# lanl-ansi/Katana.jl

Hardware: AMD Instinct MI355X
Metric: ECP iterations/sec + wall-clock to f_tol=1e-6, 1e5-var synthetic convex NLP (higher is better)
Workload: dtype f64; 1 GPU; cfg3: n=100000 variables, m_lin=50000 linear rows (8 nnz), m_nl=10000 explog rows (k=32 nnz), seed 0, planted non-degenerate vertex optimum, f_tol=1e-6; parallelism=1 GPU

## Files before the change

katana.jl_amd/csrc/engine.hpp:

```cpp
#pragma once
#include <hip/hip_runtime.h>

#include <algorithm>
#include <chrono>
#include <cstdlib>
#include <cmath>
#include <limits>
#include <map>
#include <string>
#include <vector>

#include <rccl/rccl.h>

#include "common.hpp"
#include "types.hpp"
#include "prims.hpp"

namespace ktn {

static const double kInf = std::numeric_limits<double>::infinity();

static inline int pick_group(double avg_len) {
    int g = 4;
    while (g < 64 && 2 * g <= avg_len) g <<= 1;
// ... 20 lines not shown
    int quad_group = 0;
    int esh_quad_group = 0;
    int ecp_quad_group = 0;
    int tiled_wg = 2;
    int ecp_power = 20;
    int grp_rows = 0, grp_cols = 0;
    int tiled = -1;
    double smax_reuse = 0.0;
    int power_passes = 0;
    int omega_robust = 1;
    int packed_trips = 0;
    int first_chunk = 31;
    int stag_chunk = 0;
    int near_chunk = -1;
    int stag_checks = 2;
    double flat_factor = 0.4;
    int omega_art = 1;
    double omega_art_k = 256.0;
    double omega_art_clamp = 0.0, omega_clamp = 0.0, omega_clamp_down = 0.0;
    double ipc_timeout_s = 20.0;
    bool raw_duals = false;
    int mid_refactor = 0;
    int kkt_group = 0;
    static bool flag(const char* k) { return std::getenv(k) != nullptr; }
    static int geti(const char* k, int d) { const char* v = std::getenv(k); return v ? std::atoi(v) : d; }
    static double getd(const char* k, double d) { const char* v = std::getenv(k); return v ? std::atof(v) : d; }
    void from_env() {
        no_pinned_check = flag("KTN_NO_PINNED_CHECK"); debug_load = flag("KTN_DEBUG_LOAD"); no_csc_merge = flag("KTN_NO_CSC_MERGE");
        tiled_general_build = flag("KTN_TILED_GENERAL_BUILD"); debug_blocks = flag("KTN_DEBUG_BLOCKS"); no_tiled_check = flag("KTN_NO_TILED_CHECK");
        no_setup_reuse = flag("KTN_NO_SETUP_REUSE"); debug_lp = flag("KTN_DEBUG_LP"); no_packed = flag("KTN_NO_PACKED");
        force_collective = flag("KTN_FORCE_COLLECTIVE");
        sweep_rows = geti("KTN_SWEEP_ROWS", sweep_rows); blk_cfg = geti("KTN_BLK_CFG", blk_cfg); sweep_blocked = geti("KTN_SWEEP_BLOCKED", sweep_blocked);
        sweep_batched = geti("KTN_SWEEP_BATCHED", sweep_batched); tape_classed = geti("KTN_TAPE_CLASSED", tape_classed);
        quad_group = geti("KTN_QUAD_GROUP", quad_group); esh_quad_group = geti("KTN_ESH_QUAD_GROUP", esh_quad_group);
        ecp_quad_group = geti("KTN_ECP_QUAD_GROUP", ecp_quad_group);
        tiled_wg = geti("KTN_TILED_WG", tiled_wg); ecp_power = geti("KTN_ECP_POWER", ecp_power);
        grp_rows = geti("KTN_GRP_ROWS", grp_rows); grp_cols = geti("KTN_GRP_COLS", grp_cols); tiled = geti("KTN_TILED", tiled);
        smax_reuse = getd("KTN_SMAX_REUSE", smax_reuse); power_passes = geti("KTN_POWER_PASSES", power_passes);
        omega_robust = geti("KTN_OMEGA_ROBUST", omega_robust); packed_trips = geti("KTN_PACKED_TRIPS", packed_trips);
        first_chunk = geti("KTN_FIRST_CHUNK", first_chunk); stag_chunk = geti("KTN_STAG_CHUNK", stag_chunk); near_chunk = geti("KTN_NEAR_CHUNK", near_chunk);
        stag_checks = geti("KTN_STAG_CHECKS", stag_checks); flat_factor = getd("KTN_FLAT_FACTOR", flat_factor);
        omega_art = geti("KTN_OMEGA_ART", omega_art); omega_art_k = getd("KTN_OMEGA_ART_K", omega_art_k);
        omega_art_clamp = getd("KTN_OMEGA_ART_CLAMP", omega_art_clamp); omega_clamp = getd("KTN_OMEGA_CLAMP", omega_clamp);
        omega_clamp_down = getd("KTN_OMEGA_CLAMP_DOWN", omega_clamp_down); ipc_timeout_s = getd("KTN_IPC_TIMEOUT_S", ipc_timeout_s);
        mid_refactor = geti("KTN_MID_REFACTOR", mid_refactor); raw_duals = flag("KTN_RAW_DUALS");
        kkt_group = geti("KTN_KKT_GROUP", kkt_group);
    }
};

struct Engine {
    ktn_params prm;
    DevParams dev;
    std::string err;
    hipStream_t stream = nullptr;
    int device = 0;

    bool loaded = false;
    int64_t n0 = 0, m0 = 0;
    int64_t n_lp = 0;
    int64_t m_ext = 0;
    int64_t nnz_ext = 0;
    int sense = KTN_MIN;
    bool obj_linear = true;
    bool has_inf_bound = false;
    bool has_big_bound = false;
    std::vector<int64_t> h_rowptr;
    std::vector<int32_t> h_col;
    std::vector<uint8_t> h_rowkind;
    std::vector<double> h_lb, h_ub;
// ... 410 lines not shown
    bool kkt_solved = false, kkt_arena = false, kkt_cached = false, kkt_mirror = false, kkt_seg_ok = false;
    uint64_t kkt_solves = 0, kkt_key_version = 0, kkt_key_solves = 0;
    DBuf<int32_t> d_kkt_rowmap;
    int64_t kkt_n_lin = 0;
    DBuf<int64_t> d_kkt_cptr, d_kkt_seg;
    DBuf<int32_t> d_kkt_crow, d_kkt_nonfin;
    DBuf<uint32_t> d_kkt_cperm;
    DBuf<double> d_kkt_x, d_kkt_g, d_kkt_jac, d_kkt_bconst, d_kkt_maxc, d_kkt_d, d_kkt_z, d_kkt_t, d_kkt_out, d_kkt_blk;
    std::vector<double> h_kkt_d, h_kkt_z, h_kkt_blk;
    double kkt_bound = 0.0, kkt_gap = 0.0;
    bool kkt_foreign() const { return row_sharded() || dist.cb != nullptr || dist.comm != nullptr || dist.ipc.data != nullptr || exchanging(); }
    void kkt_build_mirror();
    void kkt_compute();
    void kkt_blocks();

    void rebuild_csc();
    void purge_cuts();
    void reserve_lp(int64_t rows, int64_t nnz);
    void find_long_rows();
    bool recession_ray_dense(bool* unbounded);
    void launch_y(const SpMat& A, double sigma, double w, double rho, hipEvent_t e0, hipEvent_t e1);
    void launch_x(const SpMat& AT, double tau, double w, double rho, bool update, hipEvent_t e0, hipEvent_t e1);
    void pdhg_iteration(const SpMat& A, const SpMat& AT, double tau, double sigma, double w, double rho);
    bool launch_check(const SpMat& A, const SpMat& AT, double tau, double sigma, double w_next = -1.0, double rho = 1.0);
    DBuf<double> xnext, ynext;
    int chk_nrow = 0, chk_ncol = 0;
    void compute_scaling(bool identity);
    LpResult lp_solve(double tol_p, double tol_g, int mode, bool identity_scaling = false);
    LpResult lp_solve_core(double tol_p, double tol_g, int mode, bool identity_scaling);
    bool lp_solve_dense(LpResult* R);
    bool big_bounds_hold();
    bool lp_solve_mid(LpResult* R);
    void pdhg_raw(const double* x0, const double* y0, double eta, double omega_, int64_t iters, double* x_out,
                  double* y_out);
    void lp_resize_iterates();
    void lp_pick_groups();
    void lp_choose_tiled(bool same_matrix);
    void lp_set_anchors(bool want_packed);
    void lp_read_check(double* q);
    void lp_restart();
    void lp_advance(bool spec, int64_t k, double rho);
    struct LpScriptIO {
        const double *x, *y, *x0, *y0;
        double eta, omega;
        int64_t k;
        int32_t flags;
        const int32_t* ops;
        int64_t nops;
// ... 17 lines not shown
```

katana.jl_amd/csrc/kernels.hpp:

```cpp
#pragma once
#include <hip/hip_runtime.h>

#include <cstdint>
#include <type_traits>

#include "../../include/katana_hip.h"
#include "types.hpp"

namespace ktn {

constexpr int kKindShift = 29;
constexpr int kColMask = (1 << kKindShift) - 1;

template <int G>
__device__ __forceinline__ double group_sum(double v) {
#pragma unroll
    for (int off = G / 2; off > 0; off >>= 1) v += __shfl_xor(v, off, 64);
    return v;
}
constexpr int kLaneU = 4;
template <int U>
struct LaneBatch {
    uint32_t ix[U];
    double v[U], g[U], h[U];
// ... 29 lines not shown
#pragma unroll
    for (int u = 0; u < U; ++u)
        if (b.on[u]) acc += b.v[u] * b.g[u];
}
template <int U>
__device__ __forceinline__ void lane_add2(const LaneBatch<U>& b, double& acc, double& acc2) {
#pragma unroll
    for (int u = 0; u < U; ++u)
        if (b.on[u]) { acc += b.v[u] * b.g[u]; acc2 += b.v[u] * b.h[u]; }
}
template <int G, int U = kLaneU, class E>
__device__ __forceinline__ void lane_dot(double& acc, E beg, E len, int lane, const int32_t* __restrict__ idx, const double* __restrict__ val,
                                         const double* __restrict__ vec, int from = 0) {
    const E end = beg + len;
    for (E left = len - from - lane; left > 0; left -= U * G) {
        LaneBatch<U> b;
        lane_load<G, U>(b, end - left, end, idx, val);
        lane_gather<U>(b, vec);
        lane_add<U>(b, acc);
    }
}
template <int G, int U = kLaneU, class E>
__device__ __forceinline__ void lane_dot2(double& acc, double& acc2, E beg, E len, int lane, const int32_t* __restrict__ idx,
                                          const double* __restrict__ val, const double* __restrict__ vec, const double* __restrict__ vec2) {
    const E end = beg + len;
    for (E left = len - lane; left > 0; left -= U * G) {
        LaneBatch<U> b;
        lane_load<G, U>(b, end - left, end, idx, val);
        lane_gather2<U>(b, vec, vec2);
        lane_add2<U>(b, acc, acc2);
    }
}

template <int G>
__device__ __forceinline__ double group_max(double v) {
#pragma unroll
    for (int off = G / 2; off > 0; off >>= 1) v = fmax(v, __shfl_xor(v, off, 64));
    return v;
}
template <int G>
__device__ __forceinline__ int group_or(int v) {
#pragma unroll
    for (int off = G / 2; off > 0; off >>= 1) v |= __shfl_xor(v, off, 64);
    return v;
}
__device__ __forceinline__ double nanmax(double a, double b) {
    return (a != a || b != b) ? __builtin_nan("") : (a > b ? a : b);
}
template <int G>
// ... 1035 lines not shown
struct __attribute__((aligned(32))) ColRec { double c, l, u, x0; };
struct __attribute__((aligned(32))) RowRec { double lo, hi, y0; int32_t beg, len; };

static __global__ __launch_bounds__(kBlock) void k_pack_both(int64_t n, const int64_t* __restrict__ cptr, const double* __restrict__ c,
                                                      const double* __restrict__ l, const double* __restrict__ u, const double* __restrict__ x,
                                                      double* __restrict__ x0, ColRec* __restrict__ crec, int2* __restrict__ bl, int64_t m,
                                                      const int64_t* __restrict__ rptr, const double* __restrict__ lo, const double* __restrict__ hi,
                                                      const double* __restrict__ y, double* __restrict__ y0, RowRec* __restrict__ rrec) {
    const int64_t i = (int64_t)blockIdx.x * kBlock + threadIdx.x;
    if (i < n) {
        const double xv = x[i];
        x0[i] = xv;
        ColRec r; r.c = c[i]; r.l = l[i]; r.u = u[i]; r.x0 = xv;
        crec[i] = r;
        bl[i] = make_int2((int)cptr[i], (int)(cptr[i + 1] - cptr[i]));
    }
    if (i < m) {
        const double yv = y[i];
        y0[i] = yv;
        RowRec r; r.lo = lo[i]; r.hi = hi[i]; r.y0 = yv; r.beg = (int32_t)rptr[i]; r.len = (int32_t)(rptr[i + 1] - rptr[i]);
        rrec[i] = r;
    }
}
template <int G, int T>
__global__ __launch_bounds__(kBlock) void k_pdhg_x_packed(int64_t n, const int2* __restrict__ bl, const int32_t* __restrict__ idx,
                                                          const double* __restrict__ val, const double* __restrict__ y,
                                                          double* __restrict__ x, double* __restrict__ xbar,
                                                          const ColRec* __restrict__ rec, double tau, double w, double rho) {
    const int64_t groups = (int64_t)gridDim.x * (kBlock / G);
    const int64_t g0 = ((int64_t)blockIdx.x * kBlock + threadIdx.x) / G;
    const int lane = threadIdx.x & (G - 1);
    int2 b[T];
    ColRec r[T];
    double xv[T], acc[T];
    LaneBatch<kLaneU> lb[T];
#pragma unroll
    for (int t = 0; t < T; ++t) {
        const int64_t j = g0 + t * groups;
        b[t] = (j < n) ? bl[j] : make_int2(0, 0);
        acc[t] = 0.0;
    }
#pragma unroll
    for (int t = 0; t < T; ++t) lane_load<G, kLaneU>(lb[t], b[t].x + lane, b[t].x + b[t].y, idx, val);
#pragma unroll
    for (int t = 0; t < T; ++t) {
        const int64_t j = g0 + t * groups;
        const bool on = j < n;
        if (on) r[t] = rec[j];
        xv[t] = on ? x[j] : 0.0;
    }
#pragma unroll
    for (int t = 0; t < T; ++t) lane_gather<kLaneU>(lb[t], y);
#pragma unroll
    for (int t = 0; t < T; ++t) lane_add<kLaneU>(lb[t], acc[t]);
#pragma unroll
    for (int t = 0; t < T; ++t) lane_dot<G>(acc[t], b[t].x, b[t].y, lane, idx, val, y, kLaneU * G);
#pragma unroll
    for (int t = 0; t < T; ++t) {
        const int64_t j = g0 + t * groups;
        const double a = group_sum<G>(acc[t]);
        if (lane == 0 && j < n) {
            const double xtv = prox_x(xv[t], tau, r[t].c, a, r[t].l, r[t].u);
            xbar[j] = 2.0 * xtv - xv[t];
            x[j] = halpern(w, rho, xtv, xv[t], r[t].x0);
        }
    }
}
template <int G, int T>
__global__ __launch_bounds__(kBlock) void k_pdhg_y_packed(int64_t m, const int32_t* __restrict__ idx, const double* __restrict__ val,
                                                          const double* __restrict__ xbar, double* __restrict__ y,
                                                          const RowRec* __restrict__ rec, double sigma, double w, double rho,
                                                          int long_thresh, const int32_t* __restrict__ long_rows, int n_long) {
    const int nreg = (int)gridDim.x - n_long;
    if ((int)blockIdx.x >= nreg) {
        __shared__ double sh[kBlock / 64];
        const int i = long_rows[(int)blockIdx.x - nreg];
        const RowRec rr = rec[i];
        const int end = rr.beg + rr.len;
        double acc = 0.0;
        int e = rr.beg + (int)threadIdx.x;
        for (; e + 15 * kBlock < end; e += 16 * kBlock) {
            double v[16], xg[16];
#pragma unroll
            for (int k = 0; k < 16; ++k) v[k] = val[e + k * kBlock];
#pragma unroll
            for (int k = 0; k < 16; ++k) xg[k] = xbar[idx[e + k * kBlock]];
#pragma unroll
            for (int k = 0; k < 16; ++k) acc += v[k] * xg[k];
        }
// ... 272 lines not shown
    double xtv = 0.0, xv = 0.0, x0v = 0.0, cj = 0.0, lj = 0.0, uj = 0.0, dcj = 1.0;
    if (on) { xtv = xt[j]; xv = x[j]; x0v = x0[j]; cj = c[j]; lj = l[j]; uj = u[j]; dcj = dc[j]; }
    double aty = 0.0;
    lane_dot<G>(aty, beg, end - beg, lane, AT.idx, AT.val, yt);
    aty = group_sum<G>(aty);
    if (on && lane == 0) {
        chk_col_accumulate(a, xtv, xv, x0v, aty, cj, lj, uj, dcj);
    }
    chk_block_store<kBlock, kChkColMask, G>(a, partials);
}

template <bool UPDATE>
__global__ __launch_bounds__(kBlock) void k_x_prox(int64_t n, const double* __restrict__ aty, double* __restrict__ x,
                                                   const double* __restrict__ x0, double* __restrict__ xt, double* __restrict__ xbar,
                                                   const double* __restrict__ c, const double* __restrict__ l,
                                                   const double* __restrict__ u, double tau, double w, double rho) {
    const int64_t j = (int64_t)blockIdx.x * kBlock + threadIdx.x;
    if (j >= n) return;
    const double xv = x[j];
    const double xtv = prox_x(xv, tau, c[j], aty[j], l[j], u[j]);
    if (UPDATE) { xbar[j] = 2.0 * xtv - xv; x[j] = halpern(w, rho, xtv, xv, x0[j]); }
    else xt[j] = xtv;
}
static __global__ __launch_bounds__(kBlock) void k_chk_cols_vec(int64_t n, const double* __restrict__ atyv, const double* __restrict__ x,
                                                         const double* __restrict__ xt, const double* __restrict__ x0,
                                                         const double* __restrict__ c, const double* __restrict__ l,
                                                         const double* __restrict__ u, const double* __restrict__ dc,
                                                         double* __restrict__ partials) {
    const int64_t j = (int64_t)blockIdx.x * kBlock + threadIdx.x;
    ChkAcc a; a.init();
    if (j < n) {
        const double xtv = xt[j], xv = x[j], x0v = x0[j], cj = c[j], lj = l[j], uj = u[j], dcj = dc[j], aty = atyv[j];
        chk_col_accumulate(a, xtv, xv, x0v, aty, cj, lj, uj, dcj);
    }
    chk_block_store<kBlock, kChkColMask>(a, partials);
}

__device__ __forceinline__ double ipc_load(const double* p) {
    return __longlong_as_double((long long)__hip_atomic_load((unsigned long long*)p, __ATOMIC_RELAXED, __HIP_MEMORY_SCOPE_SYSTEM));
}
static __global__ __launch_bounds__(64) void k_ipc_barrier(IpcPeers P, int rank, int world, unsigned long long epoch, long long timeout_ticks,
                                                    int* __restrict__ err) {
    constexpr unsigned long long kPoison = ~0ULL;
    const int t = threadIdx.x;
    if (t >= world) return;
    volatile int* verr = err;
// ... 937 lines not shown
```

katana.jl_amd/csrc/lp.hip:

```cpp
#include "engine.hpp"
#include "launch.hpp"
#include "kernels.hpp"
#include "pdhg_check.hpp"
#include "dense_lp.hpp"
#include "mid_lp.hpp"
#include "batch_lp.hpp"

namespace ktn {

double Engine::dev_dot(int64_t n, const double* a, const double* b) {
    launch(k_dot_partial, kRedBlocks, kBlock, 0, stream, n, a, b, partials.p);
    launch(k_sum_final, 1, kRedBlocks, 0, stream, partials.p, kRedBlocks, chkout.p + 2 * kChkQ);
    double v = 0.0;
    KTN_HIP(hipMemcpyAsync(&v, chkout.p + 2 * kChkQ, sizeof(double), hipMemcpyDeviceToHost, stream));
    sync();
    return v;
}

double Engine::dev_finite_sq(int64_t n, const double* a) {
    launch(k_finite_sq_partial, kRedBlocks, kBlock, 0, stream, n, a, partials.p);
    launch(k_sum_final, 1, kRedBlocks, 0, stream, partials.p, kRedBlocks, chkout.p + 2 * kChkQ);
    double v = 0.0;
    KTN_HIP(hipMemcpyAsync(&v, chkout.p + 2 * kChkQ, sizeof(double), hipMemcpyDeviceToHost, stream));
    sync();
// ... 193 lines not shown
    P.max_iter = (int)std::min<int64_t>(max_it, 2000000000);
    P.nmax = blk_nmax; P.mmax = blk_mmax;
    launch(k_pdhg_blocks, (unsigned)nb, kBlkThreads, lds, stream, P);
    check_launch();
    std::vector<double> res = d_blkres.to_host(stream);
    bool all_ok = true;
    double pobj = 0.0, dobj = 0.0, pviol = 0.0, gap = 0.0, it_max = 0.0, it_sum = 0.0;
    for (int b = 0; b < nb; ++b) {
        const double* o = res.data() + (size_t)b * 8;
        if ((int)o[0] != KTN_STATUS_OPTIMAL) all_ok = false;
        pobj += o[2]; dobj += o[3]; pviol = std::max(pviol, o[4]); gap = std::max(gap, o[5]);
        it_max = std::max(it_max, o[1]); it_sum += o[1];
    }
    stats["blk_lp_launches"] += 1.0;
    stats["blk_pdhg_iters_sum"] += it_sum;
    stats["blk_pdhg_iters_max"] += it_max;
    if (!all_ok) { stats["blk_lp_fallbacks"] += 1.0; return false; }
    R->status = KTN_STATUS_OPTIMAL; R->iters = (int64_t)it_max; R->pobj = pobj; R->dobj = dobj; R->row_viol = pviol; R->gap = gap;
    return true;
}

void Engine::launch_y(const SpMat& A, double sigma, double w, double rho, hipEvent_t e0, hipEvent_t e1) {
    const int64_t m = M;
    if (m == 0) return;
    const int64_t thr = n_long > 0 ? kLongRow : (int64_t)1 << 62;
    if (tiled_on && m > 0) {
        launch_tiled(tA, m, n_lp, xbar.p, e0);
        launch_ev(k_y_epilogue, grid_n(m), kBlock, 0, stream, nullptr, e1, m, tA.pcnt.p, tpart.p, (n_long > 0 ? A.ptr : (const int64_t*)nullptr), thr, yh.p,
                  y0h.p, loh.p, hih.p, sigma, w, rho);
    } else if (packed_on) {
        const int thr32 = n_long > 0 ? (int)kLongRow : 0x7fffffff;
        const bool with_long = packed_trips != 2 && packed_trips != 4;
        with_value<2, 4, 1>(packed_trips, [&](auto t) {
            with_group(grp_rows, [&](auto g) {
                constexpr int G = g(), T = t();
                launch_ev(k_pdhg_y_packed<G, T>, T == 1 ? group_grid_long(m, G, n_long) : group_grid(m, G, T), kBlock, 0, stream, e0, e1, m, A.idx, A.val,
                          xbar.p, yh.p, d_rrec.p, sigma, w, rho, thr32, T == 1 ? (const int32_t*)d_longrows.p : nullptr, T == 1 ? (int)n_long : 0);
            });
        });
        if (with_long) return;
    } else {
        with_group(grp_rows, [&](auto g) {
            launch_timed(k_pdhg_y<g()>, group_grid(m, g()), kBlock, 0, stream, e0, e1, m, A, xbar.p, yh.p, y0h.p, loh.p, hih.p, sigma, w, rho, thr);
        });
    }
    if (n_long > 0)
        launch(k_pdhg_y_long<false>, (unsigned)n_long, kLongBlock, 0, stream, d_longrows.p, A, xbar.p, (const double*)nullptr, yh.p, y0h.p, yth.p, loh.p, hih.p,
               dr.p, sigma, w, rho, (double*)nullptr);
}

void Engine::launch_x(const SpMat& AT, double tau, double w, double rho, bool update, hipEvent_t e0, hipEvent_t e1) {
    const int64_t n = n_lp;
    if (row_sharded()) {
        const bool ipc = dist.ipc.on && n <= dist.ipc.cap;
        double* part = ipc ? ipc_slot() : pv.p;
        if (M == 0) launch_n(k_fill, n, stream, n, part, 0.0);
        if (tiled_on && M > 0) {
            launch_tiled(tAT, n, M, yh.p, e0);
            launch_ev(k_tile_vec, grid_n(n), kBlock, 0, stream, nullptr, e1, n, tAT.pcnt.p, tpart.p, part);
        }
        else spmv_cols(AT, yh.p, part, e0, e1);
        if (ipc) {
            stats["allreduce_calls"] += 1.0;
            stats["allreduce_bytes"] += 8.0 * (double)n;
            const int64_t off = ipc_barrier();
            with_bool(update, [&](auto u) {
                launch_n(k_x_prox_ipc<u()>, n, stream, n, dist.ipc.P, dist.world, off, xh.p, x0h.p, xth.p, xbar.p, ch.p, lh.p, uh.p, tau, w, rho);
            });
            return;
        }
        allreduce(pv.p, (size_t)n, 0);
        with_bool(update, [&](auto u) { launch_n(k_x_prox<u()>, n, stream, n, pv.p, xh.p, x0h.p, xth.p, xbar.p, ch.p, lh.p, uh.p, tau, w, rho); });
        return;
    }
    if (n_longc > 0 && !(tiled_on && M > 0)) {
// ... 16 lines not shown
            with_group(grp_cols, [&](auto g) {
                constexpr int G = g(), T = t();
                launch_ev(k_pdhg_x_packed<G, T>, group_grid(n, G, T), kBlock, 0, stream, e0, e1, n, d_cbl.p, AT.idx, AT.val, yh.p, xh.p, xbar.p, d_crec.p, tau, w, rho);
            });
        });
    } else {
        with_bool(update, [&](auto u) {
            constexpr bool U = u();
            with_group(grp_cols, [&](auto g) {
                launch_timed(k_pdhg_x<g(), U>, group_grid(n, g()), kBlock, 0, stream, U ? e0 : nullptr, U ? e1 : nullptr, n, AT, yh.p, xh.p, x0h.p, xth.p,
                             U ? xbar.p : nullptr, ch.p, lh.p, uh.p, tau, w, rho);
            });
        });
    }
}

void Engine::pdhg_iteration(const SpMat& A, const SpMat& AT, double tau, double sigma, double w, double rho) {
    if (!prm.profile) {
        launch_x(AT, tau, w, rho, true, nullptr, nullptr);
        launch_y(A, sigma, w, rho, nullptr, nullptr);
        return;
    }
    const int64_t n = n_lp, m = M;
    const size_t e0 = ev_get(), e1 = ev_get(), e2 = ev_get(), e3 = ev_get();
    launch_x(AT, tau, w, rho, true, ev_pool[e0], ev_pool[e1]);
    launch_y(A, sigma, w, rho, ev_pool[e2], ev_pool[e3]);
    ev_recs.push_back({0, e0, e1, (double)NNZ * 12 + 8.0 * (n + 1) + 8.0 * 7 * n + 8.0 * m});
    if (m > 0) ev_recs.push_back({1, e2, e3, (double)NNZ * 12 + 8.0 * (m + 1) + 8.0 * 5 * m + 8.0 * n});
}

bool Engine::launch_check(const SpMat& A, const SpMat& AT, double tau, double sigma, double w_next, double rho) {
    const int64_t n = n_lp, m = M;
    const int64_t thr = n_long > 0 ? kLongRow : (int64_t)1 << 62;
    const int64_t brow = group_grid(std::max<int64_t>(m, 1), grp_rows), bcol = group_grid(n, grp_cols);
    chk_part.resize((size_t)(brow + n_long + bcol) * kChkQ, stream);
    double* prow = chk_part.p;
    double* pcol = chk_part.p + (size_t)(brow + n_long) * kChkQ;
    const bool tiled_chk_off = dev.no_tiled_check;
    if (tiled_on && m > 0 && !tiled_chk_off) {
        const int64_t brow_t = grid_n(m), bcol_t = grid_n(n);
        launch_tiled(tAT, n, m, yh.p, nullptr);
        if (row_sharded()) {
            launch_n(k_tile_vec, n, stream, n, tAT.pcnt.p, tpart.p, pv.p);
            allreduce(pv.p, (size_t)n, 0);
            launch_n(k_x_prox<false>, n, stream, n, pv.p, xh.p, x0h.p, xth.p, xbar.p, ch.p, lh.p, uh.p, tau, 0.0, 1.0);
        } else {
            launch_n(k_x_epilogue_chk, n, stream, n, tAT.pcnt.p, tpart.p, xh.p, xth.p, ch.p, lh.p, uh.p, tau);
        }
        launch_tiled(tA, m, n, xth.p, nullptr);
        launch_n(k_tile_vec, m, stream, m, tA.pcnt.p, tpart.p, pw.p);
        launch_tiled(tA, m, n, xh.p, nullptr);
        launch_n(k_y_epilogue_chk, m, stream, m, tA.pcnt.p, tpart.p, pw.p, (n_long > 0 ? A.ptr : (const int64_t*)nullptr), thr, yh.p, y0h.p, yth.p, loh.p,
                 hih.p, dr.p, sigma, prow);
        if (n_long > 0)
            launch(k_pdhg_y_long<true>, (unsigned)n_long, kLongBlock, 0, stream, d_longrows.p, A, xth.p, xh.p, yh.p, y0h.p, yth.p, loh.p, hih.p, dr.p, sigma,
                   0.0, 1.0, prow + (size_t)brow_t * kChkQ);
        chk_nrow = (int)(brow_t + n_long);
        launch_tiled(tAT, n, m, yth.p, nullptr);
        launch_n(k_tile_vec, n, stream, n, tAT.pcnt.p, tpart.p, pv.p);
        if (row_sharded()) allreduce(pv.p, (size_t)n, 0);
        launch_n(k_chk_cols_vec, n, stream, n, pv.p, xh.p, xth.p, x0h.p, ch.p, lh.p, uh.p, dc.p, pcol);
        chk_ncol = (int)bcol_t;
        launch(k_chk_final, 2 * kChkQ, kRedBlocks, 0, stream, prow, chk_nrow, pcol, chk_ncol, chk_target());
        if (row_sharded()) {
            allreduce(chkout.p, 12, 0);
            allreduce(chkout.p + 12, 4, 1);
        }
        return false;
    }
    const bool spec = w_next >= 0.0 && m > 0 && !row_sharded() && n_long == 0 && n_longc == 0;
    if (spec) {
        xnext.resize((size_t)n, stream); ynext.resize((size_t)m, stream);
        with_group(grp_cols, [&](auto g) {
            launch(k_pdhg_x<g(), false>, group_grid(n, g()), kBlock, 0, stream, n, AT, yh.p, xh.p, x0h.p, xth.p, xnext.p, ch.p, lh.p, uh.p, tau, w_next, rho);
        });
    } else {
        launch_x(AT, tau, 0.0, 1.0, false, nullptr, nullptr);
    }
    if (m > 0) {
        with_group(grp_rows, [&](auto g) {
            launch(k_pdhg_y_chk<g()>, group_grid(m, g()), kBlock, 0, stream, m, A, xth.p, xh.p, yh.p, y0h.p, yth.p, loh.p, hih.p, dr.p, sigma, thr, prow,
                   spec ? ynext.p : (double*)nullptr, w_next, rho);
        });
        if (n_long > 0)
            launch(k_pdhg_y_long<true>, (unsigned)n_long, kLongBlock, 0, stream, d_longrows.p, A, xth.p, xh.p, yh.p, y0h.p, yth.p, loh.p, hih.p, dr.p, sigma,
                   0.0, 1.0, prow + (size_t)brow * kChkQ);
    }
    chk_nrow = (m > 0) ? (int)(brow + n_long) : 0;
    if (row_sharded() || n_longc > 0) {
        if (m == 0) launch_n(k_fill, n, stream, n, pv.p, 0.0);
        spmv_cols(AT, yth.p, pv.p);
        allreduce(pv.p, (size_t)n, 0);
        chk_ncol = (int)grid_n(n);
        launch_n(k_chk_cols_vec, n, stream, n, pv.p, xh.p, xth.p, x0h.p, ch.p, lh.p, uh.p, dc.p, pcol);
    } else {
        with_group(grp_cols, [&](auto g) {
            launch(k_chk_cols<g()>, group_grid(n, g()), kBlock, 0, stream, n, AT, xh.p, xth.p, x0h.p, yth.p, ch.p, lh.p, uh.p, dc.p, pcol);
        });
        chk_ncol = (int)bcol;
    }
    launch(k_chk_final, 2 * kChkQ, kRedBlocks, 0, stream, prow, chk_nrow, pcol, chk_ncol, chk_target());
    if (row_sharded()) {
        allreduce(chkout.p, 12, 0);
        allreduce(chkout.p + 12, 4, 1);
    }
    return spec;
}

LpResult Engine::lp_solve(double tol_p, double tol_g, int mode, bool identity_scaling) {
    md_y_version = 0;
    ++kkt_solves; kkt_solved = mode == 0; kkt_arena = false;
    const bool dense_ok = mode == 0 && !identity_scaling && !row_sharded() && prm.lp_dense_after != 0 && n_lp >= 1 && n_lp <= kDenseMaxN &&
                          M * n_lp <= 8000000;
    const bool mid_ok = mode == 0 && !identity_scaling && !row_sharded() && prm.lp_dense_after != 0 && n_lp > kDenseMaxN &&
                        n_lp <= std::min<int64_t>(prm.lp_mid_max_var, kMidMaxN) && n_blocks == 0 && M < ((int64_t)1 << 29);
    if (mid_ok && mid_backoff > 0) {
        --mid_backoff;
// ... 286 lines not shown
            tiled_on = build_tiled(tA, M, n_lp, lp_rowptr.p, lp_col.p, r_sval.p, kLongRow) &&
                       build_tiled(tAT, n_lp, M, c_ptr.p, c_row.p, c_sval.p, (int64_t)1 << 62);
            tpart.resize((size_t)std::max<int64_t>(tA.pieces * M, tAT.pieces * n_lp), stream);
            stats["lp_tiled_builds"] += 1.0;
            stats["lp_tiled_build_time_s"] += std::chrono::duration<double>(std::chrono::steady_clock::now() - tt).count();
            if (!tiled_on) stats["lp_tiled_overflows"] += 1.0;
        }
        tiled_built = tiled_on;
    }
}

void Engine::lp_resize_iterates() {
    const size_t n = (size_t)n_lp, mm = (size_t)std::max<int64_t>(M, 1);
    ch.resize(n, stream); lh.resize(n, stream); uh.resize(n, stream); xh.resize(n, stream);
    x0h.resize(n, stream); xth.resize(n, stream); xbar.resize(n, stream); pv.resize(n, stream);
    loh.resize(mm, stream); hih.resize(mm, stream); yh.resize(mm, stream); y0h.resize(mm, stream);
    yth.resize(mm, stream); pw.resize(mm, stream);
}

void Engine::lp_set_anchors(bool want_packed) {
    const int64_t n = n_lp, m = M;
    const size_t mm = (size_t)std::max<int64_t>(m, 1);
    packed_on = want_packed && !tiled_on && !row_sharded() && NNZ < ((int64_t)1 << 31) && !dev.no_packed;
    if (dev.packed_trips > 0) packed_trips = dev.packed_trips;
    if (packed_on) {
        d_crec.resize((size_t)n, stream); d_cbl.resize((size_t)n, stream); d_rrec.resize(mm, stream);
        launch_n(k_pack_both, std::max(n, m), stream, n, c_ptr.p, ch.p, lh.p, uh.p, xh.p, x0h.p, d_crec.p, d_cbl.p, m, lp_rowptr.p, loh.p, hih.p, yh.p, y0h.p,
                 d_rrec.p);
    } else {
        KTN_HIP(hipMemcpyAsync(x0h.p, xh.p, n * sizeof(double), hipMemcpyDeviceToDevice, stream));
        if (m > 0) KTN_HIP(hipMemcpyAsync(y0h.p, yh.p, m * sizeof(double), hipMemcpyDeviceToDevice, stream));
    }
}

void Engine::lp_read_check(double* q) {
    if (chk_pinned()) {
        sync();
        std::memcpy(q, h_chk, 2 * kChkQ * sizeof(double));
    } else {
        KTN_HIP(hipMemcpyAsync(q, chkout.p, 2 * kChkQ * sizeof(double), hipMemcpyDeviceToHost, stream));
        sync();
        ipc_check();
    }
}

void Engine::lp_restart() {
    const int64_t n = n_lp, m = M;
    launch_n(k_restart_set, std::max(n, m), stream, n, m, xth.p, xh.p, x0h.p, yth.p, yh.p, y0h.p, packed_on ? d_crec.p : (ColRec*)nullptr,
             packed_on ? d_rrec.p : (RowRec*)nullptr);
}

void Engine::lp_advance(bool spec, int64_t k, double rho) {
    const int64_t n = n_lp, m = M;
    if (spec) {
        xh.swap(xnext); yh.swap(ynext);
    } else {
        const double w = (double)(k + 1) / (double)(k + 2);
        launch_n(k_halpern2, std::max(n, m), stream, n, m, xh.p, xth.p, x0h.p, yh.p, yth.p, y0h.p, w, rho);
    }
}

LpResult Engine::lp_solve_core(double tol_p, double tol_g, int mode, bool identity_scaling) {
    auto t0 = std::chrono::steady_clock::now();
    LpResult R;
    auto lap = [&](const char* key, std::chrono::steady_clock::time_point& tp) {
        if (!prm.profile) return;
        sync();
        const auto now = std::chrono::steady_clock::now();
        stats[key] += std::chrono::duration<double>(now - tp).count();
        tp = now;
    };
    auto tp = t0;
    ensure_matrix(want_shift(mode));
    lap("lp_csc_time_s", tp);
    const bool no_reuse = dev.no_setup_reuse;
    const bool same_matrix = !no_reuse && !row_sharded() && scaled_version == lp_version && scaled_identity == identity_scaling;
// ... 153 lines not shown
    if (n_blocks > 0 && mode == 0 && !row_sharded() && n_long == 0 && m > 0 && !prm.profile) {
        if (blocks_built_rows != M) build_blocks();
        blocks_done = lp_solve_blocks(tol_p, tol_g, has_inf_bound ? eta_safe : eta, &R, max_it);
        if (blocks_done) it = R.iters;
    }
    const int near_env = dev.near_chunk;
    const int near_chunk = near_env >= 0 ? near_env : prm.lp_near_check;
    while (!blocks_done && it < max_it) {
        const double tau = eta / om, sigma = eta * om;
        if (plain_next) {
            plain_next = false;
            int want = (k <= 1 && first_chunk > 0) ? std::min(first_chunk, plain_len) : plain_len;
            if (near_conv && near_chunk > 0) want = std::min(want, near_chunk);
            if (primal_ok && stag_chunk > 0 && mode == 0) want = std::min(want, stag_chunk);
            const int np = (int)std::min<int64_t>(want, max_it - it);
            if (np <= 0) continue;
            for (int j = 0; j < np; ++j) {
                const double w = (double)(k + j + 1) / (double)(k + j + 2);
                pdhg_iteration(A, AT, tau, sigma, w, rho);
            }
            k += np; it += np;
            continue;
        }
        const bool spec_next = launch_check(A, AT, tau, sigma, (double)(k + 1) / (double)(k + 2), rho);
        check_launch();
        double q[2 * kChkQ];
        lp_read_check(q);
        if (prm.profile) ev_flush();
        const double dobj_rows = q[2], yt2 = q[4];
        const PdhgSums S{q[0], q[1], q[3], q[kChkQ + 5], q[kChkQ + 8], q[kChkQ + 9], yt2,
                         q[kChkQ + 6] + obj_shift, dobj_rows + q[kChkQ + 7] + obj_shift, q[12], q[kChkQ + 13]};
        const PdhgStop t = pdhg_stop(S, rules, pc, om, eta, k);
        if (dbg_lp) std::fprintf(stderr, "[lp mode %d] it %7lld k %6lld r %.3e pviol %.3e dres %.3e gap %.3e pobj %.10g dobj %.10g om %.3g eta %.3g\n",
                                 mode, (long long)it, (long long)k, t.r, S.pviol, S.dres, t.gap, S.pobj, S.dobj, om, eta);
        R.pobj = S.pobj; R.dobj = S.dobj; R.row_viol = S.pviol; R.gap = t.gap;
        R.dres_rel = S.dres / rules.dres_scale;
        near_conv = t.near; primal_ok = t.primal_ok;
        if (t.exit != PDHG_EXIT_NONE) {
            if (t.exit == PDHG_EXIT_STAGNATION) { R.stag_exit = true; stats["lp_stagnation_exits"] += 1.0; }
            if (t.exit == PDHG_EXIT_STALLED_ROW) stats["lp_stalled_row_exits"] += 1.0;
            R.status = t.exit == PDHG_EXIT_NAN ? KTN_STATUS_ERROR : KTN_STATUS_OPTIMAL;
            ++it;
            break;
        }
        if (mode == 0 && (m > 0 || row_sharded())) {
            const double farkas = dobj_rows + q[kChkQ + 10];
            const double mag = q[10] + q[kChkQ + 11] + 1e-300;
            const bool cert = farkas > 1e-6 * mag && q[kChkQ + 14] <= 1e-9 * (1.0 + std::sqrt(yt2)) && S.pviol > tol_p;
            infeas_hits = cert ? infeas_hits + 1 : 0;
            if (infeas_hits >= 2 && it >= 2 * chk) {
                R.status = KTN_STATUS_INFEASIBLE;
                ++it;
                break;
            }
        }
        const PdhgNext nx = pdhg_next(S, rules, pc, t, om, eta, k, it);
        if (nx.backoff != PDHG_BACKOFF_NONE) stats["lp_eta_backoffs"] += 1.0;
        if (nx.backoff == PDHG_BACKOFF_GROW) stats["lp_divergence_backoffs"] += 1.0;
        eta = nx.eta;
        if (nx.action == PDHG_CONSOLIDATE) {
            stats["lp_consolidations"] += 1.0;
            launch_n(k_unscale, n, stream, n, xth.p, dc.p, pv.p);
            SpMat Au{lp_rowptr.p, lp_col.p, Wval()};
            with_group(grp_rows, [&](auto g) { launch(k_spmv<g()>, group_grid(m, g()), kBlock, 0, stream, m, Au, pv.p, pw.p); });
            KTN_HIP(hipMemsetAsync(d_anynf.p + 1, 0, sizeof(int32_t), stream));
            launch_n(k_consolidate, list_count(), stream, list_count(), list_heads(), d_cutprev.p, pw.p, Wlo(), Whi(), dr.p, tol_p, yth.p, d_anynf.p + 1);
        }
        if (nx.action != PDHG_ADVANCE) {
            if (nx.action == PDHG_RESTART) {
                if (dbg_lp) std::fprintf(stderr, "[lp restart] it %lld k %lld decayed %d dx %.3e dy %.3e |xt| %.3e |yt| %.3e om %.4g\n", (long long)it, (long long)k, (int)(t.r <= 0.8 * pc.r0), std::sqrt(S.dx0sq), std::sqrt(S.dy0sq), std::sqrt(S.xt2), std::sqrt(S.yt2), om);
                stats["lp_restarts"] += 1.0;
            }
            om = nx.om;
            if (nx.backoff == PDHG_BACKOFF_GROW && has_inf_bound) {
                launch_n(k_cold_point, std::max(n, m), stream, n, m, lh.p, uh.p, xth.p, yth.p);
                eta = eta_safe;
                om = om_start;
                stats["lp_cold_restarts"] += 1.0;
            }
            lp_restart();
            k = 0;
            ++it;
            continue;
        }
        lp_advance(spec_next, k, rho);
        ++k; ++it;
        plain_next = true;
    }
    R.iters = it;
    if (mode == 0) {
        launch_n(k_unscale2, std::max(n, m), stream, n, xth.p, dc.p, lp_x.p, m, yth.p, dr.p, lp_y.p);
        if (w_shift) {
            epi_dot(lp_x.p);
            launch(k_epi_var, 1, 1, 0, stream, lp_x.p, (int32_t)n0, epi_scal.p, (const double*)nullptr, 1, 0, sgn, epi_newest.p);
        }
        omega = om;
        have_omega = true;
        objval = sgn * R.pobj + c0;
    } else {
        launch_n(k_unscale, n, stream, n, xth.p, dc.p, d_ray.p);
    }
    check_launch();
    sync();
    if (prm.profile) ev_flush();
    stats["pdhg_iters"] += (double)it;
    stats["lp_solves"] += 1.0;
    stats["lp_last_row_viol"] = R.row_viol; stats["lp_last_gap"] = R.gap; stats["lp_last_dres_rel"] = R.dres_rel;
    stats["lp_last_stag_exit"] = R.stag_exit ? 1.0 : 0.0;
    stats["lp_time_s"] += std::chrono::duration<double>(std::chrono::steady_clock::now() - t0).count();
    return R;
}

void Engine::pdhg_raw(const double* x0, const double* y0, double eta, double omega_, int64_t iters, double* x_out,
                      double* y_out) {
    ensure_matrix(false);
    compute_scaling(true);
    scaled_version = 0;
    const int64_t n = n_lp, m = M;
    lp_resize_iterates();
    const double sgn = (sense == KTN_MAX) ? -1.0 : 1.0;
    KTN_HIP(hipMemcpyAsync(lp_x.p, x0, n * sizeof(double), hipMemcpyHostToDevice, stream));
    if (m > 0) KTN_HIP(hipMemcpyAsync(lp_y.p, y0, m * sizeof(double), hipMemcpyHostToDevice, stream));
    launch_n(k_prep_cols, n, stream, n, lp_c.p, lp_l.p, lp_u.p, dc.p, lp_x.p, (double*)nullptr, sgn, 0, ch.p, lh.p, uh.p, xh.p);
    launch_n(k_prep_rows, m, stream, m, lp_lo.p, lp_hi.p, dr.p, lp_y.p, 0, loh.p, hih.p, yh.p);
    grp_rows = pick_group(m ? (double)NNZ / (double)m : 1.0);
    grp_cols = pick_group(n ? (double)NNZ / (double)n : 1.0);
    SpMat A{lp_rowptr.p, lp_col.p, r_sval.p};
    SpMat AT{c_ptr.p, c_row.p, c_sval.p};
    packed_on = false;
    KTN_HIP(hipMemcpyAsync(x0h.p, xh.p, n * sizeof(double), hipMemcpyDeviceToDevice, stream));
    if (m > 0) KTN_HIP(hipMemcpyAsync(y0h.p, yh.p, m * sizeof(double), hipMemcpyDeviceToDevice, stream));
    find_long_rows();
    lp_choose_tiled(false);
    const double tau = eta / omega_, sigma = eta * omega_;
    for (int64_t k = 0; k < iters; ++k) {
        const double w = (double)(k + 1) / (double)(k + 2);
        pdhg_iteration(A, AT, tau, sigma, w, 1.0);
        if ((k & 255) == 255) { sync(); if (prm.profile) ev_flush(); }
    }
    sync();
    if (prm.profile) ev_flush();
    check_launch();
    KTN_HIP(hipMemcpyAsync(x_out, xh.p, n * sizeof(double), hipMemcpyDeviceToHost, stream));
    if (m > 0) KTN_HIP(hipMemcpyAsync(y_out, yh.p, m * sizeof(double), hipMemcpyDeviceToHost, stream));
    sync();
}

void Engine::lp_script(const LpScriptIO& io) {
    const bool identity = (io.flags & KTN_LPS_IDENTITY) != 0;
    ensure_matrix(false);
    find_long_rows();
    scal_rows = 0;
// ... 17 lines not shown
    prep(io.x, io.y);
    check_launch();
    stats["lp_long_rows"] = (double)n_long; stats["lp_long_cols"] = (double)n_longc;
    stats["lp_packed"] = packed_on ? 1.0 : 0.0; stats["lp_packed_trips"] = (double)packed_trips;
    stats["lp_grp_rows"] = (double)grp_rows; stats["lp_grp_cols"] = (double)grp_cols;
    stats["lp_tiled"] = tiled_on ? 1.0 : 0.0;
    stats["lp_tiled_check"] = (tiled_on && m > 0 && !dev.no_tiled_check) ? 1.0 : 0.0;
    stats["lp_tiled_pieces"] = tiled_on ? (double)std::max(tA.pieces, tAT.pieces) : 0.0;
    stats["lp_check_pinned"] = chk_pinned() ? 1.0 : 0.0;
    const double tau = io.eta / io.omega, sigma = io.eta * io.omega, rho = 1.0;
    int64_t k = io.k;
    bool checked = false, spec = false;
    double q[2 * kChkQ];
    for (int q_ = 0; q_ < 2 * kChkQ; ++q_) q[q_] = 0.0;
    for (int64_t o = 0; o < io.nops; ++o) {
        const double w = (double)(k + 1) / (double)(k + 2);
        switch (io.ops[o]) {
            case KTN_LPOP_STEP:
                launch_x(AT, tau, w, rho, true, nullptr, nullptr);
                launch_y(A, sigma, w, rho, nullptr, nullptr);
                ++k; checked = false;
                break;
            case KTN_LPOP_CHECK:
                spec = launch_check(A, AT, tau, sigma, (io.flags & KTN_LPS_NO_SPEC) ? -1.0 : w, rho);
                check_launch();
                lp_read_check(q);
                if (spec && io.xnext_out) xnext.download(io.xnext_out, (size_t)n, stream);
                if (spec && io.ynext_out && m > 0) ynext.download(io.ynext_out, (size_t)m, stream);
                checked = true;
                break;
            case KTN_LPOP_ADVANCE:
                KTN_REQUIRE(checked, "lp_script: advance without a check before it");
                lp_advance(spec, k, rho);
                ++k; checked = false;
                break;
            case KTN_LPOP_RESTART:
                KTN_REQUIRE(checked, "lp_script: restart without a check before it");
                lp_restart();
                k = 0; checked = false;
                break;
            default:
                KTN_REQUIRE(false, "lp_script: unknown op");
        }
        if ((o & 255) == 255) sync();
    }
    check_launch();
    sync();
// ... 77 lines not shown
```

Before: 363.6 ECP iterations/s.

## Fuse next PDHG x-step into convergence check column pass and reuse Aᵀy after restart

During a speculative check with packed columns, the column-check pass is merged with the following iteration's x-update. One packed kernel computes both Aᵀ·ynext and Aᵀ·ythat, writes the look-ahead x and xbar, and accumulates the check partials. On advance the precomputed x is swapped in instead of relaunching the x SpMV. After a restart, the stored Aᵀy is reused so the speculative x needs only an elementwise kernel. This removes one sparse transpose pass per check cycle, at the cost of extra buffers, state tracking, and invalidation logic that must stay consistent with restarts, cuts and cold points.

```diff
diff --git a/katana.jl_amd/csrc/engine.hpp b/katana.jl_amd/csrc/engine.hpp
--- a/katana.jl_amd/csrc/engine.hpp
+++ b/katana.jl_amd/csrc/engine.hpp
@@ -66,6 +66,7 @@
     bool raw_duals = false;
     int mid_refactor = 0;
     int kkt_group = 0;
+    int check_ride = 1;
     static bool flag(const char* k) { return std::getenv(k) != nullptr; }
     static int geti(const char* k, int d) { const char* v = std::getenv(k); return v ? std::atoi(v) : d; }
     static double getd(const char* k, double d) { const char* v = std::getenv(k); return v ? std::atof(v) : d; }
@@ -88,7 +89,7 @@
         omega_art_clamp = getd("KTN_OMEGA_ART_CLAMP", omega_art_clamp); omega_clamp = getd("KTN_OMEGA_CLAMP", omega_clamp);
         omega_clamp_down = getd("KTN_OMEGA_CLAMP_DOWN", omega_clamp_down); ipc_timeout_s = getd("KTN_IPC_TIMEOUT_S", ipc_timeout_s);
         mid_refactor = geti("KTN_MID_REFACTOR", mid_refactor); raw_duals = flag("KTN_RAW_DUALS");
-        kkt_group = geti("KTN_KKT_GROUP", kkt_group);
+        kkt_group = geti("KTN_KKT_GROUP", kkt_group); check_ride = geti("KTN_CHECK_RIDE", check_ride);
     }
 };
 
@@ -545,8 +546,14 @@
     void launch_y(const SpMat& A, double sigma, double w, double rho, hipEvent_t e0, hipEvent_t e1);
     void launch_x(const SpMat& AT, double tau, double w, double rho, bool update, hipEvent_t e0, hipEvent_t e1);
     void pdhg_iteration(const SpMat& A, const SpMat& AT, double tau, double sigma, double w, double rho);
-    bool launch_check(const SpMat& A, const SpMat& AT, double tau, double sigma, double w_next = -1.0, double rho = 1.0);
+    bool launch_check(const SpMat& A, const SpMat& AT, double tau, double sigma, double w_next = -1.0, double rho = 1.0, double w_ahead = -1.0);
     DBuf<double> xnext, ynext;
+    DBuf<double> x_ahead, xbar_ahead, aty_t;
+    bool ahead_made = false, ahead_armed = false;
+    double ahead_tau = 0.0, ahead_w = 0.0, ahead_rho = 0.0;
+    int aty_state = 0;
+    void ride_reset() { ahead_made = ahead_armed = false; aty_state = 0; }
+    bool take_ahead(double tau, double w, double rho);
     int chk_nrow = 0, chk_ncol = 0;
     void compute_scaling(bool identity);
     LpResult lp_solve(double tol_p, double tol_g, int mode, bool identity_scaling = false);
diff --git a/katana.jl_amd/csrc/kernels.hpp b/katana.jl_amd/csrc/kernels.hpp
--- a/katana.jl_amd/csrc/kernels.hpp
+++ b/katana.jl_amd/csrc/kernels.hpp
@@ -75,9 +75,10 @@
 }
 template <int G, int U = kLaneU, class E>
 __device__ __forceinline__ void lane_dot2(double& acc, double& acc2, E beg, E len, int lane, const int32_t* __restrict__ idx,
-                                          const double* __restrict__ val, const double* __restrict__ vec, const double* __restrict__ vec2) {
+                                          const double* __restrict__ val, const double* __restrict__ vec, const double* __restrict__ vec2,
+                                          int from = 0) {
     const E end = beg + len;
-    for (E left = len - lane; left > 0; left -= U * G) {
+    for (E left = len - from - lane; left > 0; left -= U * G) {
         LaneBatch<U> b;
         lane_load<G, U>(b, end - left, end, idx, val);
         lane_gather2<U>(b, vec, vec2);
@@ -1159,17 +1160,25 @@
         rrec[i] = r;
     }
 }
-template <int G, int T>
-__global__ __launch_bounds__(kBlock) void k_pdhg_x_packed(int64_t n, const int2* __restrict__ bl, const int32_t* __restrict__ idx,
-                                                          const double* __restrict__ val, const double* __restrict__ y,
-                                                          double* __restrict__ x, double* __restrict__ xbar,
-                                                          const ColRec* __restrict__ rec, double tau, double w, double rho) {
+__device__ __forceinline__ void chk_col_accumulate(ChkAcc& a, double xtv, double xv, double x0v, double aty, double cj, double lj,
+                                                   double uj, double dcj);
+template <int G, int T, bool RIDE>
+__device__ __forceinline__ void pdhg_x_packed_body(int64_t n, const int2* __restrict__ bl, const int32_t* __restrict__ idx,
+                                                   const double* __restrict__ val, const double* __restrict__ y,
+                                                   double* __restrict__ x, double* __restrict__ xbar,
+                                                   const ColRec* __restrict__ rec, double tau, double w, double rho,
+                                                   const double* __restrict__ yt, const double* __restrict__ xt,
+                                                   const double* __restrict__ xk, const double* __restrict__ dc,
+                                                   double* __restrict__ x_ahead, double* __restrict__ xbar_ahead,
+                                                   double* __restrict__ aty_t, double* __restrict__ partials) {
+    static_assert(!RIDE || T == 1, "the ride form serves one column per lane group");
     const int64_t groups = (int64_t)gridDim.x * (kBlock / G);
     const int64_t g0 = ((int64_t)blockIdx.x * kBlock + threadIdx.x) / G;
     const int lane = threadIdx.x & (G - 1);
     int2 b[T];
     ColRec r[T];
     double xv[T], acc[T];
+    double xtc = 0.0, xkc = 0.0, dcj = 1.0, aty = 0.0;
     LaneBatch<kLaneU> lb[T];
 #pragma unroll
     for (int t = 0; t < T; ++t) {
@@ -1185,23 +1194,66 @@
         const bool on = j < n;
         if (on) r[t] = rec[j];
         xv[t] = on ? x[j] : 0.0;
-    }
-#pragma unroll
-    for (int t = 0; t < T; ++t) lane_gather<kLaneU>(lb[t], y);
-#pragma unroll
-    for (int t = 0; t < T; ++t) lane_add<kLaneU>(lb[t], acc[t]);
-#pragma unroll
-    for (int t = 0; t < T; ++t) lane_dot<G>(acc[t], b[t].x, b[t].y, lane, idx, val, y, kLaneU * G);
+        if constexpr (RIDE) {
+            if (on) { xtc = xt[j]; xkc = xk[j]; dcj = dc[j]; }
+        }
+    }
+    if constexpr (RIDE) {
+        lane_gather2<kLaneU>(lb[0], y, yt);
+        lane_add2<kLaneU>(lb[0], acc[0], aty);
+        lane_dot2<G>(acc[0], aty, b[0].x, b[0].y, lane, idx, val, y, yt, kLaneU * G);
+    } else {
+#pragma unroll
+        for (int t = 0; t < T; ++t) lane_gather<kLaneU>(lb[t], y);
+#pragma unroll
+        for (int t = 0; t < T; ++t) lane_add<kLaneU>(lb[t], acc[t]);
+#pragma unroll
+        for (int t = 0; t < T; ++t) lane_dot<G>(acc[t], b[t].x, b[t].y, lane, idx, val, y, kLaneU * G);
+    }
 #pragma unroll
     for (int t = 0; t < T; ++t) {
         const int64_t j = g0 + t * groups;
         const double a = group_sum<G>(acc[t]);
         if (lane == 0 && j < n) {
             const double xtv = prox_x(xv[t], tau, r[t].c, a, r[t].l, r[t].u);
-            xbar[j] = 2.0 * xtv - xv[t];
-            x[j] = halpern(w, rho, xtv, xv[t], r[t].x0);
-        }
-    }
+            if constexpr (RIDE) {
+                xbar_ahead[j] = 2.0 * xtv - xv[t];
+                x_ahead[j] = halpern(w, rho, xtv, xv[t], r[t].x0);
+            } else {
+                xbar[j] = 2.0 * xtv - xv[t];
+                x[j] = halpern(w, rho, xtv, xv[t], r[t].x0);
+            }
+        }
+    }
+    if constexpr (RIDE) {
+        ChkAcc ca; ca.init();
+        aty = group_sum<G>(aty);
+        if (lane == 0 && g0 < n) {
+            aty_t[g0] = aty;
+            chk_col_accumulate(ca, xtc, xkc, r[0].x0, aty, r[0].c, r[0].l, r[0].u, dcj);
+        }
+        chk_block_store<kBlock, kChkColMask, G>(ca, partials);
+    }
+}
+template <int G, int T>
+__global__ __launch_bounds__(kBlock) void k_pdhg_x_packed(int64_t n, const int2* __restrict__ bl, const int32_t* __restrict__ idx,
+                                                          const double* __restrict__ val, const double* __restrict__ y,
+                                                          double* __restrict__ x, double* __restrict__ xbar,
+                                                          const ColRec* __restrict__ rec, double tau, double w, double rho) {
+    pdhg_x_packed_body<G, T, false>(n, bl, idx, val, y, x, xbar, rec, tau, w, rho, nullptr, nullptr, nullptr, nullptr, nullptr, nullptr, nullptr,
+                                    nullptr);
+}
+template <int G>
+__global__ __launch_bounds__(kBlock) void k_pdhg_x_packed_ride(int64_t n, const int2* __restrict__ bl, const int32_t* __restrict__ idx,
+                                                               const double* __restrict__ val, const double* __restrict__ ynext,
+                                                               const double* __restrict__ xnext, const ColRec* __restrict__ rec,
+                                                               double tau, double w, double rho, const double* __restrict__ yt,
+                                                               const double* __restrict__ xt, const double* __restrict__ xk,
+                                                               const double* __restrict__ dc, double* __restrict__ x_ahead,
+                                                               double* __restrict__ xbar_ahead, double* __restrict__ aty_t,
+                                                               double* __restrict__ partials) {
+    pdhg_x_packed_body<G, 1, true>(n, bl, idx, val, ynext, const_cast<double*>(xnext), nullptr, rec, tau, w, rho, yt, xt, xk, dc, x_ahead, xbar_ahead,
+                                   aty_t, partials);
 }
 template <int G, int T>
 __global__ __launch_bounds__(kBlock) void k_pdhg_y_packed(int64_t m, const int32_t* __restrict__ idx, const double* __restrict__ val,
@@ -1520,6 +1572,17 @@
     if (UPDATE) { xbar[j] = 2.0 * xtv - xv; x[j] = halpern(w, rho, xtv, xv, x0[j]); }
     else xt[j] = xtv;
 }
+static __global__ __launch_bounds__(kBlock) void k_pdhg_x_aty(int64_t n, const double* __restrict__ aty, const double* __restrict__ x,
+                                                       const double* __restrict__ x0, double* __restrict__ xt, double* __restrict__ xnext,
+                                                       const double* __restrict__ c, const double* __restrict__ l,
+                                                       const double* __restrict__ u, double tau, double w, double rho) {
+    const int64_t j = (int64_t)blockIdx.x * kBlock + threadIdx.x;
+    if (j >= n) return;
+    const double xv = x[j];
+    const double xtv = prox_x(xv, tau, c[j], aty[j], l[j], u[j]);
+    xt[j] = xtv;
+    xnext[j] = halpern(w, rho, xtv, xv, x0[j]);
+}
 static __global__ __launch_bounds__(kBlock) void k_chk_cols_vec(int64_t n, const double* __restrict__ atyv, const double* __restrict__ x,
                                                          const double* __restrict__ xt, const double* __restrict__ x0,
                                                          const double* __restrict__ c, const double* __restrict__ l,
diff --git a/katana.jl_amd/csrc/lp.hip b/katana.jl_amd/csrc/lp.hip
--- a/katana.jl_amd/csrc/lp.hip
+++ b/katana.jl_amd/csrc/lp.hip
@@ -239,6 +239,7 @@
 
 void Engine::launch_y(const SpMat& A, double sigma, double w, double rho, hipEvent_t e0, hipEvent_t e1) {
     const int64_t m = M;
+    aty_state = 0;
     if (m == 0) return;
     const int64_t thr = n_long > 0 ? kLongRow : (int64_t)1 << 62;
     if (tiled_on && m > 0) {
@@ -266,8 +267,18 @@
                dr.p, sigma, w, rho, (double*)nullptr);
 }
 
+bool Engine::take_ahead(double tau, double w, double rho) {
+    const bool hit = ahead_armed && tau == ahead_tau && w == ahead_w && rho == ahead_rho;
+    ahead_made = ahead_armed = false;
+    if (!hit) return false;
+    xh.swap(x_ahead); xbar.swap(xbar_ahead);
+    stats["lp_check_ride_hits"] += 1.0;
+    return true;
+}
+
 void Engine::launch_x(const SpMat& AT, double tau, double w, double rho, bool update, hipEvent_t e0, hipEvent_t e1) {
     const int64_t n = n_lp;
+    if (update && take_ahead(tau, w, rho)) return;
     if (row_sharded()) {
         const bool ipc = dist.ipc.on && n <= dist.ipc.cap;
         double* part = ipc ? ipc_slot() : pv.p;
@@ -330,15 +341,20 @@
         return;
     }
     const int64_t n = n_lp, m = M;
-    const size_t e0 = ev_get(), e1 = ev_get(), e2 = ev_get(), e3 = ev_get();
-    launch_x(AT, tau, w, rho, true, ev_pool[e0], ev_pool[e1]);
+    if (!take_ahead(tau, w, rho)) {
+        const size_t e0 = ev_get(), e1 = ev_get();
+        launch_x(AT, tau, w, rho, true, ev_pool[e0], ev_pool[e1]);
+        ev_recs.push_back({0, e0, e1, (double)NNZ * 12 + 8.0 * (n + 1) + 8.0 * 7 * n + 8.0 * m});
+    }
+    const size_t e2 = ev_get(), e3 = ev_get();
     launch_y(A, sigma, w, rho, ev_pool[e2], ev_pool[e3]);
-    ev_recs.push_back({0, e0, e1, (double)NNZ * 12 + 8.0 * (n + 1) + 8.0 * 7 * n + 8.0 * m});
     if (m > 0) ev_recs.push_back({1, e2, e3, (double)NNZ * 12 + 8.0 * (m + 1) + 8.0 * 5 * m + 8.0 * n});
 }
 
-bool Engine::launch_check(const SpMat& A, const SpMat& AT, double tau, double sigma, double w_next, double rho) {
+bool Engine::launch_check(const SpMat& A, const SpMat& AT, double tau, double sigma, double w_next, double rho, double w_ahead) {
     const int64_t n = n_lp, m = M;
+    const bool aty_is_aty = aty_state == 2;
+    ride_reset();
     const int64_t thr = n_long > 0 ? kLongRow : (int64_t)1 << 62;
     const int64_t brow = group_grid(std::max<int64_t>(m, 1), grp_rows), bcol = group_grid(n, grp_cols);
     chk_part.resize((size_t)(brow + n_long + bcol) * kChkQ, stream);
@@ -377,11 +393,17 @@
         return false;
     }
     const bool spec = w_next >= 0.0 && m > 0 && !row_sharded() && n_long == 0 && n_longc == 0;
+    const bool ride = spec && packed_on && packed_trips == 1 && dev.check_ride != 0 && w_ahead >= 0.0;
     if (spec) {
         xnext.resize((size_t)n, stream); ynext.resize((size_t)m, stream);
-        with_group(grp_cols, [&](auto g) {
-            launch(k_pdhg_x<g(), false>, group_grid(n, g()), kBlock, 0, stream, n, AT, yh.p, xh.p, x0h.p, xth.p, xnext.p, ch.p, lh.p, uh.p, tau, w_next, rho);
-        });
+        if (ride && aty_is_aty && aty_t.n == (size_t)n) {
+            launch_n(k_pdhg_x_aty, n, stream, n, aty_t.p, xh.p, x0h.p, xth.p, xnext.p, ch.p, lh.p, uh.p, tau, w_next, rho);
+            stats["lp_restart_reuses"] += 1.0;
+        } else {
+            with_group(grp_cols, [&](auto g) {
+                launch(k_pdhg_x<g(), false>, group_grid(n, g()), kBlock, 0, stream, n, AT, yh.p, xh.p, x0h.p, xth.p, xnext.p, ch.p, lh.p, uh.p, tau, w_next, rho);
+            });
+        }
     } else {
         launch_x(AT, tau, 0.0, 1.0, false, nullptr, nullptr);
     }
@@ -401,6 +423,16 @@
         allreduce(pv.p, (size_t)n, 0);
         chk_ncol = (int)grid_n(n);
         launch_n(k_chk_cols_vec, n, stream, n, pv.p, xh.p, xth.p, x0h.p, ch.p, lh.p, uh.p, dc.p, pcol);
+    } else if (ride) {
+        x_ahead.resize((size_t)n, stream); xbar_ahead.resize((size_t)n, stream); aty_t.resize((size_t)n, stream);
+        with_group(grp_cols, [&](auto g) {
+            launch(k_pdhg_x_packed_ride<g()>, group_grid(n, g()), kBlock, 0, stream, n, d_cbl.p, AT.idx, AT.val, ynext.p, xnext.p, d_crec.p, tau, w_ahead, rho,
+                   yth.p, xth.p, xh.p, dc.p, x_ahead.p, xbar_ahead.p, aty_t.p, pcol);
+        });
+        chk_ncol = (int)bcol;
+        ahead_made = true; ahead_tau = tau; ahead_w = w_ahead; ahead_rho = rho;
+        aty_state = 1;
+        stats["lp_check_rides"] += 1.0;
     } else {
         with_group(grp_cols, [&](auto g) {
             launch(k_chk_cols<g()>, group_grid(n, g()), kBlock, 0, stream, n, AT, xh.p, xth.p, x0h.p, yth.p, ch.p, lh.p, uh.p, dc.p, pcol);
@@ -733,6 +765,7 @@
     const int64_t n = n_lp, m = M;
     const size_t mm = (size_t)std::max<int64_t>(m, 1);
     packed_on = want_packed && !tiled_on && !row_sharded() && NNZ < ((int64_t)1 << 31) && !dev.no_packed;
+    ride_reset();
     if (dev.packed_trips > 0) packed_trips = dev.packed_trips;
     if (packed_on) {
         d_crec.resize((size_t)n, stream); d_cbl.resize((size_t)n, stream); d_rrec.resize(mm, stream);
@@ -759,10 +792,15 @@
     const int64_t n = n_lp, m = M;
     launch_n(k_restart_set, std::max(n, m), stream, n, m, xth.p, xh.p, x0h.p, yth.p, yh.p, y0h.p, packed_on ? d_crec.p : (ColRec*)nullptr,
              packed_on ? d_rrec.p : (RowRec*)nullptr);
+    ahead_made = ahead_armed = false;
+    aty_state = aty_state == 1 ? 2 : 0;
 }
 
 void Engine::lp_advance(bool spec, int64_t k, double rho) {
     const int64_t n = n_lp, m = M;
+    ahead_armed = spec && ahead_made;
+    ahead_made = false;
+    aty_state = 0;
     if (spec) {
         xh.swap(xnext); yh.swap(ynext);
     } else {
@@ -962,7 +1000,7 @@
             k += np; it += np;
             continue;
         }
-        const bool spec_next = launch_check(A, AT, tau, sigma, (double)(k + 1) / (double)(k + 2), rho);
+        const bool spec_next = launch_check(A, AT, tau, sigma, (double)(k + 1) / (double)(k + 2), rho, (double)(k + 2) / (double)(k + 3));
         check_launch();
         double q[2 * kChkQ];
         lp_read_check(q);
@@ -1005,6 +1043,7 @@
             with_group(grp_rows, [&](auto g) { launch(k_spmv<g()>, group_grid(m, g()), kBlock, 0, stream, m, Au, pv.p, pw.p); });
             KTN_HIP(hipMemsetAsync(d_anynf.p + 1, 0, sizeof(int32_t), stream));
             launch_n(k_consolidate, list_count(), stream, list_count(), list_heads(), d_cutprev.p, pw.p, Wlo(), Whi(), dr.p, tol_p, yth.p, d_anynf.p + 1);
+            aty_state = 0;
         }
         if (nx.action != PDHG_ADVANCE) {
             if (nx.action == PDHG_RESTART) {
@@ -1014,6 +1053,7 @@
             om = nx.om;
             if (nx.backoff == PDHG_BACKOFF_GROW && has_inf_bound) {
                 launch_n(k_cold_point, std::max(n, m), stream, n, m, lh.p, uh.p, xth.p, yth.p);
+                aty_state = 0;
                 eta = eta_safe;
                 om = om_start;
                 stats["lp_cold_restarts"] += 1.0;
@@ -1028,6 +1068,7 @@
         plain_next = true;
     }
     R.iters = it;
+    ride_reset();
     if (mode == 0) {
         launch_n(k_unscale2, std::max(n, m), stream, n, xth.p, dc.p, lp_x.p, m, yth.p, dr.p, lp_y.p);
         if (w_shift) {
@@ -1068,6 +1109,7 @@
     SpMat A{lp_rowptr.p, lp_col.p, r_sval.p};
     SpMat AT{c_ptr.p, c_row.p, c_sval.p};
     packed_on = false;
+    ride_reset();
     KTN_HIP(hipMemcpyAsync(x0h.p, xh.p, n * sizeof(double), hipMemcpyDeviceToDevice, stream));
     if (m > 0) KTN_HIP(hipMemcpyAsync(y0h.p, yh.p, m * sizeof(double), hipMemcpyDeviceToDevice, stream));
     find_long_rows();
@@ -1131,7 +1173,7 @@
                 ++k; checked = false;
                 break;
             case KTN_LPOP_CHECK:
-                spec = launch_check(A, AT, tau, sigma, (io.flags & KTN_LPS_NO_SPEC) ? -1.0 : w, rho);
+                spec = launch_check(A, AT, tau, sigma, (io.flags & KTN_LPS_NO_SPEC) ? -1.0 : w, rho, (double)(k + 2) / (double)(k + 3));
                 check_launch();
                 lp_read_check(q);
                 if (spec && io.xnext_out) xnext.download(io.xnext_out, (size_t)n, stream);
```

Result: slower. 357.2 ECP iterations/s (-1.7%).
